# MrTornado24/FENeRF

Measured on NVIDIA H100. Metric: rendered faces/sec at 128px x 24 samples/ray, higher is better.
Workload: dtype f16 operands / f32 accumulate (wgmma) + f32 refinement

## Files before the change

fenerf_b200/_lib.py:

```python
import ctypes as C
import os

_HERE = os.path.dirname(os.path.abspath(__file__))
LIB_PATH = os.environ.get("FENERF_B200_LIB") or os.path.join(_HERE, "libfenerf_b200.so")

MAX_TRUNK, MAX_COLOR, MAX_LABEL, HIDDEN = 8, 8, 32, 256

ABI_VERSION = 3
FIELD_LABEL_FILM = 0x1
FIELD_FEATURE_HEAD = 0x8
PRECISION = {"exact": 0, "fast": 1, "guard": 2}
CLAMP = {"relu": 0, "softplus": 1}
FILL_MODE = {None: 0, "debug": 1, "weight": 2, "weight_debug": 3, "seg_padding_background": 4,
             "eval_seg_padding_background": 5, "eval_white_back": 6}
FILL_COLOR = {"black": 0.0, "white": 1.0, "grey": 0.5, "light_grey": 0.81}
E_CLAMP_MODE = -5
CAMERA_MODE = {"uniform": 1, "normal": 2, "gaussian": 2, "truncated_gaussian": 3, "spherical_uniform": 4}

EXPORTS = (
    "fenerf_packed_bytes", "fenerf_pack_field", "fenerf_siren_points", "fenerf_ray_setup", "fenerf_resample",
    "fenerf_composite", "fenerf_workspace_bytes", "fenerf_render_forward", "fenerf_last_error",
    "fenerf_abi_version", "fenerf_launch_count", "fenerf_camera_poses",
    "fenerf_field_fingerprint", "fenerf_composite_backward", "fenerf_film_forward_stash", "fenerf_gate_backward",
    "fenerf_head_grads", "fenerf_extras_gather", "fenerf_grid_scatter_add", "fenerf_grid_unpack_grad",
    "fenerf_workspace_layout", "fenerf_mask2color", "fenerf_frames_to_u8", "fenerf_mapping_film",
    "fenerf_guard_stats", "fenerf_debug_stage_times", "fenerf_gemm_nt_f16", "fenerf_gemm_nt_film", "fenerf_gemm_tn_f16",
)


class FieldDesc(C.Structure):
    _fields_ = [("trunk_layers", C.c_int32), ("color_layers", C.c_int32), ("label_dim", C.c_int32),
                ("grid_channels", C.c_int32), ("grid_res", C.c_int32), ("out_dim", C.c_int32),
                ("input_scale", C.c_float), ("reserved", C.c_int32)]


class FieldParams(C.Structure):
    _fields_ = [("trunk_w", C.c_void_p * MAX_TRUNK), ("trunk_b", C.c_void_p * MAX_TRUNK),
                ("sigma_w", C.c_void_p), ("sigma_b", C.c_void_p),
                ("color_w", C.c_void_p * MAX_COLOR), ("color_b", C.c_void_p * MAX_COLOR),
                ("rgb_w", C.c_void_p), ("rgb_b", C.c_void_p),
                ("label_w", C.c_void_p * 3), ("label_b", C.c_void_p * 3),
                ("grid", C.c_void_p)]


class RenderDesc(C.Structure):
    _fields_ = [("batch", C.c_int32), ("img_h", C.c_int32), ("img_w", C.c_int32), ("num_steps", C.c_int32),
                ("hierarchical", C.c_int32), ("clamp_mode", C.c_int32),
                ("last_back", C.c_int32), ("white_back", C.c_int32), ("black_back", C.c_int32),
                ("fill_mode", C.c_int32), ("fill_color", C.c_float), ("softmax_label", C.c_int32),
                ("lock_view_dependence", C.c_int32), ("precision", C.c_int32),
                ("noise_std", C.c_float), ("tan_half_fov", C.c_float), ("guard_tau", C.c_float)]


class GuardReport(C.Structure):
    _fields_ = [("refined", C.c_int32), ("max_abs_delta", C.c_float), ("sign_flips", C.c_int32), ("tau", C.c_float)]


class MappingParams(C.Structure):
    _fields_ = [("weight", C.c_void_p * 5), ("bias", C.c_void_p * 5), ("z_dim", C.c_int32), ("hidden_dim", C.c_int32)]
# ... 24 lines not shown
    lib.fenerf_ray_setup.argtypes = [P(RenderDesc)] + [vp] * 10
    lib.fenerf_resample.restype = C.c_int
    lib.fenerf_resample.argtypes = [P(RenderDesc), i32] + [vp] * 10
    lib.fenerf_composite.restype = C.c_int
    lib.fenerf_composite.argtypes = [P(RenderDesc), i32] + [vp] * 11
    lib.fenerf_workspace_bytes.restype = sz
    lib.fenerf_workspace_bytes.argtypes = [P(RenderDesc), P(FieldDesc)]
    lib.fenerf_workspace_layout.restype = C.c_int
    lib.fenerf_workspace_layout.argtypes = [P(RenderDesc), P(FieldDesc), P(WorkspaceOffsets)]
    lib.fenerf_render_forward.restype = C.c_int
    lib.fenerf_render_forward.argtypes = [P(RenderDesc), P(FieldDesc)] + [vp] * 15 + [vp, sz, vp]
    lib.fenerf_composite_backward.restype = C.c_int
    lib.fenerf_composite_backward.argtypes = [P(RenderDesc), i32] + [vp] * 9
    lib.fenerf_film_forward_stash.restype = C.c_int
    lib.fenerf_film_forward_stash.argtypes = [vp, vp, vp, i64, i64, i64, vp, i32, vp, vp, vp, i32, vp]
    lib.fenerf_gate_backward.restype = C.c_int
    lib.fenerf_gate_backward.argtypes = [vp, vp, i64, i64, vp, i32, vp]
    lib.fenerf_head_grads.restype = C.c_int
    lib.fenerf_head_grads.argtypes = [vp, vp, i64, i32, i32, vp, vp, vp, i32, vp]
    lib.fenerf_extras_gather.restype = C.c_int
    lib.fenerf_extras_gather.argtypes = [P(FieldDesc), vp, vp, vp, i64, i64, i32, i32, vp, vp]
    lib.fenerf_grid_scatter_add.restype = C.c_int
    lib.fenerf_grid_scatter_add.argtypes = [P(FieldDesc), vp, vp, i32, i64, vp, i32, vp]
    lib.fenerf_grid_unpack_grad.restype = C.c_int
    lib.fenerf_grid_unpack_grad.argtypes = [P(FieldDesc), vp, vp, vp, vp]
    lib.fenerf_gemm_nt_f16.restype = C.c_int
    lib.fenerf_gemm_nt_f16.argtypes = [vp, vp, i64, vp, vp, vp, vp]
    lib.fenerf_gemm_nt_film.restype = C.c_int
    lib.fenerf_gemm_nt_film.argtypes = [vp, vp, i64, vp, vp, i64, i64, vp, vp, vp, vp, vp]
    lib.fenerf_gemm_tn_f16.restype = C.c_int
    lib.fenerf_gemm_tn_f16.argtypes = [vp, vp, i32, i64, i32, vp, vp, vp]
    lib.fenerf_debug_stage_times.restype = C.c_int
    lib.fenerf_debug_stage_times.argtypes = [i32, vp]
    lib.fenerf_guard_stats.restype = C.c_int
    lib.fenerf_guard_stats.argtypes = [vp, P(GuardReport), vp]
    lib.fenerf_mapping_film.restype = C.c_int
    lib.fenerf_mapping_film.argtypes = [P(MappingParams), vp, i32, i32, i32, i32, vp, vp, C.c_float, vp, vp, vp]
    lib.fenerf_mask2color.restype = C.c_int
    lib.fenerf_mask2color.argtypes = [vp, i32, i32, i64, vp, vp]
    lib.fenerf_frames_to_u8.restype = C.c_int
    lib.fenerf_frames_to_u8.argtypes = [vp, i32, i32, i32, i32, i64, vp, vp]
    lib.fenerf_last_error.restype = C.c_char_p
    lib.fenerf_last_error.argtypes = []
    lib.fenerf_abi_version.restype = i32
    lib.fenerf_abi_version.argtypes = []
    lib.fenerf_launch_count.restype = i64
    lib.fenerf_launch_count.argtypes = []


def lib():
    global _lib
    if _lib is None:
        if not os.path.exists(LIB_PATH):
            raise RuntimeError(
                "libfenerf_b200.so is missing (%s): run `python -m fenerf_b200.build` or "
                "__graft_entry__.build(); the render path has no CPU / PyTorch fallback" % LIB_PATH)
        handle = C.CDLL(LIB_PATH)
        _declare(handle)
        if handle.fenerf_abi_version() != ABI_VERSION:
            raise RuntimeError("libfenerf_b200.so ABI version mismatch")
        _lib = handle
    return _lib


class FenerfError(RuntimeError):
    def __init__(self, code, message):
# ... 15 lines not shown
```

fenerf_b200/csrc/abi.cu:

```cuda
#include "common.cuh"
#include <stdlib.h>

namespace fn {
thread_local char g_err[512] = "";
std::atomic<long long> g_launches{0};
}

using namespace fn;

namespace {

struct Workspace {
    size_t stats, points_c, z_c, dirs, origins, raw_c, z_f, points_f, raw_f, guard, sigma_c, total;
};

Workspace plan_workspace(const fenerf_render_desc* rd, int C) {
    Workspace w;
    size_t n_rays = (size_t)rd->batch * rd->img_h * rd->img_w;
    size_t pc = n_rays * rd->num_steps;
    size_t off = 0;
    auto take = [&](size_t bytes) { size_t o = off; off = fn_align_up(off + bytes, 256); return o; };
    w.stats = take(64);
    w.points_c = take(pc * 3 * 4);
    w.z_c = take(pc * 4);
// ... 146 lines not shown
}

int fenerf_composite(const fenerf_render_desc* rd, int32_t out_dim, const float* raw_coarse, const float* z_coarse,
                     const float* raw_fine, const float* z_fine, const float* rng_noise, float* pixels, float* depth,
                     float* weights_sum, float* weights, int32_t* sort_idx, void* stream) {
    if (int e = check_render_desc(rd)) return e;
    FN_REQUIRE(raw_coarse && z_coarse && pixels, "NULL argument");
    FN_REQUIRE(rd->noise_std == 0.f || rng_noise, "noise_std != 0 needs rng_noise");
    return composite(rd, out_dim, raw_coarse, z_coarse, raw_fine, z_fine, rd->noise_std != 0.f ? rng_noise : nullptr,
                     pixels, depth, weights_sum, weights, sort_idx, (cudaStream_t)stream);
}

size_t fenerf_workspace_bytes(const fenerf_render_desc* rd, const fenerf_field_desc* field) {
    if (!rd || !field) return 0;
    return plan_workspace(rd, field->out_dim).total;
}

int fenerf_debug_stage_times(int32_t enable, float* ms_out) {
    if (enable && !g_stage_timing) {
        for (int i = 0; i <= kStages; ++i) FN_CUDA_OK(cudaEventCreate(&g_stage_ev[i]));
        g_stage_timing = true;
        return 0;
    }
    if (!enable && g_stage_timing) {
        g_stage_timing = false;
        for (int i = 0; i <= kStages; ++i) cudaEventDestroy(g_stage_ev[i]);
        return 0;
    }
    if (g_stage_timing && ms_out) {
        FN_CUDA_OK(cudaEventSynchronize(g_stage_ev[kStages]));
        for (int i = 0; i < kStages; ++i) FN_CUDA_OK(cudaEventElapsedTime(ms_out + i, g_stage_ev[i], g_stage_ev[i + 1]));
    }
    return 0;
}

int fenerf_guard_stats(const void* workspace, fenerf_guard_report* out, void* stream) {
    FN_REQUIRE(workspace && out, "NULL argument");
    int32_t raw[4];
    FN_CUDA_OK(cudaMemcpyAsync(raw, workspace, sizeof(raw), cudaMemcpyDeviceToHost, (cudaStream_t)stream));
    FN_CUDA_OK(cudaStreamSynchronize((cudaStream_t)stream));
    out->refined = raw[0];
    out->max_abs_delta = *reinterpret_cast<const float*>(&raw[1]);
    out->sign_flips = raw[2];
    out->tau = *reinterpret_cast<const float*>(&raw[3]);
    return 0;
}

int fenerf_workspace_layout(const fenerf_render_desc* rd, const fenerf_field_desc* field, fenerf_workspace_offsets* out) {
    if (int e = check_render_desc(rd)) return e;
    FN_REQUIRE(field && out, "NULL argument");
    Workspace w = plan_workspace(rd, field->out_dim);
    out->points_coarse = w.points_c; out->z_coarse = w.z_c; out->dirs = w.dirs; out->origins = w.origins;
    out->raw_coarse = w.raw_c; out->z_fine = w.z_f; out->points_fine = w.points_f; out->raw_fine = w.raw_f;
    out->total = w.total;
    return 0;
}

int fenerf_render_forward(const fenerf_render_desc* rd, const fenerf_field_desc* field, const void* packed,
                          const float* film, const float* x_lin, const float* y_lin, const float* z_lin,
                          const float* cam2world, const float* rng_perturb, const float* rng_noise_c,
                          const float* rng_u, const float* rng_noise_f, float* pixels, float* depth,
                          float* weights_sum, float* weights, int64_t* inds_dbg, void* workspace,
                          size_t workspace_bytes, void* stream) {
    if (int e = check_render_desc(rd)) return e;
    FnLayout L;
    FnLabelFilm lf;
// ... 173 lines not shown
```

fenerf_b200/csrc/common.cuh:

```cuda
#pragma once
#include <cuda_runtime.h>
#include <cuda_fp16.h>
#include <stdarg.h>
#include <stdint.h>
#include <stdio.h>
#include <atomic>

#include "../../include/fenerf_b200.h"
#include "layout.h"

namespace fn {

extern thread_local char g_err[512];
extern std::atomic<long long> g_launches;

inline int fail(int code, const char* fmt, ...) {
    va_list ap;
    va_start(ap, fmt);
    vsnprintf(g_err, sizeof(g_err), fmt, ap);
    va_end(ap);
    return code;
}

inline void count_launch(int n = 1) { g_launches.fetch_add(n, std::memory_order_relaxed); }
// ... 44 lines not shown
    const int dev = current_device();
    if (state[dev].load(std::memory_order_acquire) >= bytes) return cudaSuccess;
    cudaError_t e = cudaFuncSetAttribute(kernel, cudaFuncAttributeMaxDynamicSharedMemorySize, bytes);
    if (e == cudaSuccess) state[dev].store(bytes, std::memory_order_release);
    return e;
}

constexpr float kFarDelta = 1e10f;

__device__ __forceinline__ float softplus_torch(float x) { return x > 20.f ? x : log1pf(expf(x)); }

__device__ __forceinline__ float density_act(float sigma, int clamp_mode) {
    return clamp_mode == FENERF_CLAMP_RELU ? fmaxf(sigma, 0.f) : softplus_torch(sigma);
}

__device__ __forceinline__ float sample_alpha(float delta, float act, float* decay = nullptr) {
    const float e = expf(__fmul_rn(-delta, act));
    if (decay) *decay = e;
    return __fsub_rn(1.f, e);
}

__device__ __forceinline__ float transmittance_term(float alpha) { return __fadd_rn(__fsub_rn(1.f, alpha), 1e-10f); }

int pack_field(const fenerf_field_desc* f, const FnLayout& L, const FnLabelFilm& lf, const FnFeatureHead& fh,
               const fenerf_field_params* p, void* packed, cudaStream_t st);
int siren_points_exact(const FnLayout& L, const FnLabelFilm& lf, const FnFeatureHead& fh, const unsigned char* packed,
                       const float* points, const float* dirs, const float* film, int batch, long long ppb, int dir_group,
                       int lock_dirs, const int32_t* only_idx, int n_only, float* out, cudaStream_t st, int sigma_only = 0);
int field_fingerprint(const FnLayout& L, const FnLabelFilm& lf, const FnFeatureHead& fh, const fenerf_field_params* p,
                      unsigned long long* out, cudaStream_t st);
int siren_points_fast(const FnLayout& L, const FnLabelFilm& lf, const FnFeatureHead& fh, const unsigned char* packed,
                      const float* points, const float* dirs, const float* film, int batch, long long ppb, int dir_group,
                      int lock_dirs, float* out, int sigma_only, cudaStream_t st, float* sigma_out = nullptr);
int guard_refine(const FnLayout& L, const unsigned char* packed, const float* points, const float* dirs,
                 const float* film, int batch, long long rays_per_batch, int num_steps, int lock_dirs, float tau,
                 const float* noise_far, long long noise_stride, float noise_std,
                 float* raw, int32_t* scratch_idx, int32_t* stats, cudaStream_t st);
int camera_poses(int n, int mode, float h_std, float v_std, float h_mean, float v_mean, const float* draw_theta,
                 const float* draw_phi, float* c2w, float* pitch, float* yaw, cudaStream_t st);
int ray_setup(const fenerf_render_desc* rd, const float* x_lin, const float* y_lin, const float* z_lin,
              const float* cam2world, const float* rng_perturb, float* points, float* z_vals, float* dirs,
              float* origins, cudaStream_t st);
int resample(const fenerf_render_desc* rd, int C, const float* raw, const float* z, const float* dirs,
             const float* origins, const float* noise, const float* u, float* z_fine, float* pts_fine,
             long long* inds, cudaStream_t st, int sort_fine = 0, const float* sigma_compact = nullptr);
int composite_sorted(const fenerf_render_desc* rd, int C, const float* raw_c, const float* z_c, const float* raw_f,
                     const float* z_f, const float* noise, float* pixels, float* depth, float* wsum, float* weights,
                     cudaStream_t st);
int composite(const fenerf_render_desc* rd, int C, const float* raw_c, const float* z_c, const float* raw_f,
              const float* z_f, const float* noise, float* pixels, float* depth, float* wsum, float* weights,
              int32_t* sort_idx, cudaStream_t st);
int composite_backward(const fenerf_render_desc* rd, int C, const float* raw_c, const float* z_c, const float* raw_f,
                       const float* z_f, const float* noise, const float* d_pixels, float* d_raw_c, float* d_raw_f,
                       cudaStream_t st);

int gemm_nt(const void* A, const void* B, long long M, float* c32, void* c16, void* a_out, void* gate_out, const float* bias,
            const float* film, long long film_stride, long long ppb, cudaStream_t st, const void* gate_mul = nullptr,
            const void* A2 = nullptr, const void* B2 = nullptr);
int gemm_tn(const void* X, const void* Y, int batch, long long ppb, int slices, float* partial, cudaStream_t st,
            float* colsum = nullptr);
int mapping_film(const float* const* w, const float* const* b, const float* z, int B, int z_dim, int n_layers, int layer0,
                 int n_film_total, const float* avg_f, const float* avg_p, float psi, float* h_scratch, float* film,
                 cudaStream_t st);
int mask2color(const float* masks, int B, int K, long long HW, float* out, cudaStream_t st);
int frames_to_u8(const float* frames, int B, int C, int c0, int nc, long long HW, unsigned char* out, cudaStream_t st);
int film_forward_stash(const float* z, const float* bias, const float* film_layer, long long film_batch_stride, long long P,
// ... 13 lines not shown
```

fenerf_b200/csrc/siren_fast.cu:

```cuda
#include "siren_fast.cuh"

namespace fn {

int siren_fast_label_launch(const void* args, int blocks, cudaStream_t st);
int siren_fast_hd_launch(const void* args, int blocks, bool label_film, cudaStream_t st);

namespace {

bool build_loads(const FnLayout& L, const FnLabelFilm& lf, const FnFeatureHead& fh, FastArgs& A, bool sigma_only) {
    A.n_loads = 0;
    auto push = [&](size_t src, uint32_t bytes) {
        if (A.n_loads < MAX_LOADS) A.loads[A.n_loads] = Load{(uint32_t)src, bytes};
        ++A.n_loads;
    };
    push(L.first_img, 2 * CHUNK);
    for (int l = 0; l < L.n_hidden; ++l) {
        if (l == L.trunk_hidden) {
            push(L.head_img, 4 * HEAD_CHUNK);
            if (sigma_only) return A.n_loads <= MAX_LOADS;
        }
        if (lf.on && l == lf.layer) {
            push(L.hid_img[l], 2 * CHUNK);
            push(L.hid_img[l] + 2 * CHUNK, 2 * CHUNK);
            if (fh.on) push(fh.label_img, 4 * FEAT_CHUNK);
            else push(lf.img, 4 * HEAD_CHUNK);
            push(L.hid_img[l] + 4 * CHUNK, 2 * CHUNK);
            push(L.hid_img[l] + 6 * CHUNK, 2 * CHUNK);
            continue;
        }
        push(L.hid_img[l], 2 * CHUNK);
        push(L.hid_img[l] + 2 * CHUNK, 2 * CHUNK);
        if (l == L.trunk_hidden + lf.on) push(L.color0_ximg, 2 * CHUNK);
        push(L.hid_img[l] + 4 * CHUNK, 2 * CHUNK);
        push(L.hid_img[l] + 6 * CHUNK, 2 * CHUNK);
    }
    if (fh.on) push(fh.rgb_img, 4 * FEAT_CHUNK);
    else push(L.rgb_img, 4 * RGB_CHUNK);
    return A.n_loads <= MAX_LOADS;
}

}

int siren_points_fast(const FnLayout& L_in, const FnLabelFilm& lf_in, const FnFeatureHead& fh_in, const unsigned char* packed,
                      const float* points, const float* dirs, const float* film, int batch, long long ppb, int dir_group,
                      int lock_dirs, float* out, int sigma_only, cudaStream_t st, float* sigma_out) {
    static_assert(sizeof(FastArgs) <= 4000, "kernel parameter block too large");
    static_assert(SMEM_TOTAL <= 232448, "one CTA per SM: 227 KB of shared memory");
    static_assert(4 * FEAT_CHUNK == SLOT_BYTES, "a feature-head image is one ring slot");
    const FnFeatureHead no_fh = {0, 0, 0, 0, 0};
    const FnLabelFilm no_lf = {0, 0, 0};
    const bool trunk_only = fh_in.on && sigma_only;
    const FnFeatureHead& fh = trunk_only ? no_fh : fh_in;
    const FnLabelFilm& lf = trunk_only ? no_lf : lf_in;
    const FnLayout L = fh.on ? fn_head_view(L_in, fh) : fn_trunk_view(L_in, fh_in);
    FN_REQUIRE(L.trunk_hidden >= 1 && L.n_hidden - L.trunk_hidden - lf.on >= 1, "field needs >= 2 trunk and >= 1 colour layers");
    FN_REQUIRE(fh.on || L.label_dim < 32, "the fast path packs labels and sigma into one 32-column head (label_dim <= 31)");
    FN_REQUIRE(L.rgb_img < 0xFFFFFFFFull && lf.img < 0xFFFFFFFFull && fh.rgb_img < 0xFFFFFFFFull && fh.label_img < 0xFFFFFFFFull,
               "packed weight images beyond 4 GB");
    FN_REQUIRE(((uintptr_t)film & 15) == 0, "the FiLM table must be 16-byte aligned");
    FastArgs a;
    memset(&a, 0, sizeof(a));
    FN_REQUIRE(build_loads(L, lf, fh, a, sigma_only != 0), "field too deep for the weight stream");
    a.sigma_only = sigma_only ? 1 : 0;
    a.L = L; a.packed = packed; a.points = points; a.dirs = dirs; a.film = film; a.out = out; a.sigma_out = sigma_out;
    a.ppb = ppb; a.tiles_per_batch = (ppb + TILE - 1) / TILE; a.n_tiles = a.tiles_per_batch * batch;
    a.dir_group = dir_group < 1 ? 1 : dir_group; a.lock_dirs = lock_dirs;
    if (a.n_tiles <= 0) return 0;
    FN_REQUIRE(ppb % a.dir_group == 0, "points_per_batch %lld not a multiple of dir_group %d", ppb, a.dir_group);
    const long long n_pairs = (a.n_tiles + 1) / 2;
    static std::atomic<int> attr_set[kMaxDevices];
    const int blocks = (int)(n_pairs < (long long)num_sms() ? n_pairs : (long long)num_sms());
    if (fh.on) return siren_fast_hd_launch(&a, blocks, lf.on != 0, st);
    if (lf.on) return siren_fast_label_launch(&a, blocks, st);
    FN_CUDA_OK(ensure_dynamic_smem(siren_fast_kernel<false>, attr_set, (int)SMEM_TOTAL));
    siren_fast_kernel<false><<<blocks, NTHREADS, SMEM_TOTAL, st>>>(a);
    FN_LAUNCH_OK("siren_fast_kernel");
    return 0;
}

}
```

fenerf_b200/csrc/siren_fast.cuh:

```cuda
#pragma once
#include "common.cuh"
#include "siren_common.cuh"
#include "sm90.cuh"

namespace fn {

namespace {

using namespace sm90;

constexpr int TILE = 64;
constexpr int NTHREADS = 384;
constexpr int PROD_WARP = 8;
constexpr int RING = 6;
constexpr uint32_t SLOT_BYTES = 32768;
constexpr int XSTRIDE = 72;
constexpr uint32_t SMEM_X = RING * SLOT_BYTES;
constexpr int FRING = 2;
constexpr uint32_t FILM_BYTES = 3 * FN_H * 4;
constexpr uint32_t SMEM_FILM = SMEM_X + 2 * TILE * XSTRIDE * 2;
constexpr uint32_t SMEM_BAR = SMEM_FILM + 2 * FRING * FILM_BYTES;
constexpr uint32_t SMEM_TOTAL = SMEM_BAR + 16 * RING + 16 + 16 * 2 * FRING;
constexpr int MAX_LOADS = 72;
constexpr uint32_t CHUNK = 16384;
constexpr uint32_t HEAD_CHUNK = 32 * 128;
constexpr uint32_t RGB_CHUNK = 8 * 128;
constexpr uint32_t FEAT_CHUNK = FN_FEAT * 128;

struct Load {
    uint32_t src;
    uint32_t bytes;
};

struct FastArgs {
    Load loads[MAX_LOADS];
    int n_loads;
    FnLayout L;
    const unsigned char* packed;
    const float* points;
    const float* dirs;
    const float* film;
    float* out;
    float* sigma_out;
    long long ppb, tiles_per_batch, n_tiles;
    int dir_group, lock_dirs;
    int sigma_only;
};

__device__ __forceinline__ void wg_bar(int wg) { asm volatile("bar.sync %0, 128;" ::"r"(1 + wg) : "memory"); }

template <bool kLabelFilm, bool kFeatureHead = false>
__global__ void __launch_bounds__(NTHREADS, 1) siren_fast_kernel(const __grid_constant__ FastArgs a) {
    extern __shared__ __align__(1024) unsigned char smem[];
    const uint32_t sbase = smem_u32(smem);
    const int warp = threadIdx.x >> 5, lane = threadIdx.x & 31;
    const uint32_t bar_full = sbase + SMEM_BAR, bar_empty = bar_full + 8 * RING, bar_turn = bar_empty + 8 * RING;
    const uint32_t bar_ffull = bar_turn + 16, bar_fempty = bar_ffull + 8 * 2 * FRING;
    if (threadIdx.x == 0) {
        for (int i = 0; i < RING; ++i) {
            mbar_init(bar_full + 8 * i, 1);
            mbar_init(bar_empty + 8 * i, 8);
        }
        for (int g = 0; g < 2; ++g) mbar_init(bar_turn + 8 * g, 4);
        for (int e = 0; e < 2 * FRING; ++e) {
            mbar_init(bar_ffull + 8 * e, 1);
            mbar_init(bar_fempty + 8 * e, 4);
        }
        fence_barrier_init();
    }
    __syncthreads();
    const long long n_pairs = (a.n_tiles + 1) / 2;

    if (warp >= PROD_WARP) {
        asm volatile("setmaxnreg.dec.sync.aligned.u32 40;\n" ::: "memory");
        if (warp == PROD_WARP && lane == 0) {
            uint32_t it = 0;
            for (long long pair = blockIdx.x; pair < n_pairs; pair += gridDim.x)
                for (int i = 0; i < a.n_loads; ++i, ++it) {
                    const uint32_t slot = it % RING;
                    mbar_wait(bar_empty + 8 * slot, ((it / RING) & 1u) ^ 1u);
                    mbar_arrive_expect_tx(bar_full + 8 * slot, a.loads[i].bytes);
                    bulk_g2s(sbase + slot * SLOT_BYTES, a.packed + a.loads[i].src, a.loads[i].bytes, bar_full + 8 * slot);
                }
        } else if ((warp == PROD_WARP + 1 || warp == PROD_WARP + 2) && lane == 0) {
            const int g = warp - PROD_WARP - 1;
            const int n_film = 1 + (a.sigma_only ? a.L.trunk_hidden : a.L.n_hidden);
            uint32_t it = 0;
            for (long long pair = blockIdx.x; pair < n_pairs; pair += gridDim.x) {
                const long long tile = pair * 2 + g;
                const long long b = tile < a.n_tiles ? tile / a.tiles_per_batch : 0;
                const float* film_b = a.film + (size_t)b * a.L.n_film * 2 * FN_H;
                for (int i = 0; i < n_film; ++i, ++it) {
                    const uint32_t e = g * FRING + it % FRING;
                    const uint32_t dst = sbase + SMEM_FILM + e * FILM_BYTES;
                    mbar_wait(bar_fempty + 8 * e, ((it / FRING) & 1u) ^ 1u);
                    mbar_arrive_expect_tx(bar_ffull + 8 * e, FILM_BYTES);
                    bulk_g2s(dst, film_b + (size_t)i * 2 * FN_H, 2 * FN_H * 4, bar_ffull + 8 * e);
                    bulk_g2s(dst + 2 * FN_H * 4, a.packed + (i == 0 ? a.L.first_b : a.L.hid_b[i - 1]), FN_H * 4, bar_ffull + 8 * e);
                }
            }
        }
        return;
    }

    asm volatile("setmaxnreg.inc.sync.aligned.u32 232;\n" ::: "memory");
    const int wg = warp >> 2, q = lane & 3;
    const int tid = threadIdx.x & 127;
    const int r0 = (warp & 3) * 16 + (lane >> 2);
    const FnLayout& L = a.L;
    const int C = L.out_dim;
    const float* sigma_w = reinterpret_cast<const float*>(a.packed + L.sigma_w);
    const float* rgb_w = reinterpret_cast<const float*>(a.packed + L.rgb_w);
    const float* label_w = reinterpret_cast<const float*>(a.packed + L.label_w);
    __half* xs = reinterpret_cast<__half*>(smem + SMEM_X) + wg * TILE * XSTRIDE;
    uint32_t it = 0;
    auto acquire = [&](uint32_t& slot) -> uint32_t {
        slot = it % RING;
        mbar_wait(bar_full + 8 * slot, (it / RING) & 1u);
        ++it;
        return sbase + slot * SLOT_BYTES;
    };
    auto release = [&](uint32_t slot) {
        __syncwarp();
        if (lane == 0) mbar_arrive(bar_empty + 8 * slot);
    };
    uint32_t turns = 0;
    uint32_t fit = 0;
    auto film_acquire = [&]() -> const float* {
        const uint32_t e = wg * FRING + fit % FRING;
        mbar_wait(bar_ffull + 8 * e, (fit / FRING) & 1u);
        return reinterpret_cast<const float*>(smem + SMEM_FILM + e * FILM_BYTES);
    };
    auto film_release = [&]() {
        const uint32_t e = wg * FRING + fit % FRING;
        ++fit;
        __syncwarp();
        if (lane == 0) mbar_arrive(bar_fempty + 8 * e);
    };
    auto turn_begin = [&]() { mbar_wait(bar_turn + 8 * wg, (turns & 1u) ^ (wg == 0 ? 1u : 0u)); };
    auto turn_end = [&]() {
        ++turns;
        __syncwarp();
        if (lane == 0) mbar_arrive(bar_turn + 8 * (wg ^ 1));
    };
    auto xfrag = [&](int s, uint32_t (&f)[4]) {
        const __half* p = xs + r0 * XSTRIDE + 16 * s + 2 * q;
        f[0] = *reinterpret_cast<const uint32_t*>(p);
        f[1] = *reinterpret_cast<const uint32_t*>(p + 8 * XSTRIDE);
        f[2] = *reinterpret_cast<const uint32_t*>(p + 8);
        f[3] = *reinterpret_cast<const uint32_t*>(p + 8 * XSTRIDE + 8);
    };

    for (long long pair = blockIdx.x; pair < n_pairs; pair += gridDim.x) {
        const long long tile = pair * 2 + wg;
        const bool tile_ok = tile < a.n_tiles;
        const long long b = tile_ok ? tile / a.tiles_per_batch : 0;
        const long long p0 = tile_ok ? (tile % a.tiles_per_batch) * TILE : a.ppb;

        wg_bar(wg);
        if (tid < TILE) {
            float pos[3] = {0.f, 0.f, 0.f}, dir[3] = {0.f, 0.f, 0.f};
            const long long pp = p0 + tid;
            const bool valid = pp < a.ppb;
            if (valid) {
                const long long ff = b * a.ppb + pp;
#pragma unroll
                for (int i = 0; i < 3; ++i) pos[i] = __fmul_rn(a.points[ff * 3 + i], L.input_scale);
                if (a.lock_dirs) dir[2] = -1.f;
                else {
                    const long long di = b * (a.ppb / a.dir_group) + pp / a.dir_group;
#pragma unroll
                    for (int i = 0; i < 3; ++i) dir[i] = a.dirs[di * 3 + i];
                }
            }
            __align__(16) __half slots[64];
#pragma unroll
            for (int i = 0; i < 64; ++i) slots[i] = __float2half_rn(0.f);
#pragma unroll
            for (int i = 0; i < 3; ++i) {
                __half hi, lo;
                split_f16(pos[i], hi, lo);
                slots[FN_SLOT_POS + i] = hi; slots[FN_SLOT_POS + 3 + i] = lo; slots[FN_SLOT_POS + 6 + i] = hi;
                split_f16(dir[i], hi, lo);
                slots[FN_SLOT_DIR + i] = hi; slots[FN_SLOT_DIR + 3 + i] = lo; slots[FN_SLOT_DIR + 6 + i] = hi;
            }
            if (L.grid_channels > 0 && valid && !a.sigma_only) {
                float feat[32];
                grid_features32_h(reinterpret_cast<const __half*>(a.packed + L.grid16), L.grid_res, pos[0], pos[1], pos[2], feat);
#pragma unroll
                for (int i = 0; i < 32; ++i) slots[FN_SLOT_FEAT + i] = __float2half_rn(feat[i]);
            }
#pragma unroll
            for (int i = 0; i < 8; ++i)
                reinterpret_cast<uint4*>(xs + tid * XSTRIDE)[i] = reinterpret_cast<const uint4*>(slots)[i];
        }
        wg_bar(wg);

        uint32_t act[16][4];
        uint32_t nxt[8][4];
        float d[64];
        auto film_epi = [&](const float* fs, int h, uint32_t (&dst)[8][4]) {
            const float* fl = fs + h * 128;
            const float* bias = fs + 2 * FN_H + h * 128;
#pragma unroll
            for (int j = 0; j < 16; ++j) {
                const int c = 8 * j + 2 * q;
                const float2 fr = *reinterpret_cast<const float2*>(fl + c);
                const float2 ph = *reinterpret_cast<const float2*>(fl + FN_H + c);
                const float2 bi = *reinterpret_cast<const float2*>(bias + c);
                const float px = fmaf(fr.x, bi.x, ph.x), py = fmaf(fr.y, bi.y, ph.y);
                dst[j >> 1][(j & 1) * 2] = pack_half2(__sinf(fmaf(fr.x, d[4 * j], px)), __sinf(fmaf(fr.y, d[4 * j + 1], py)));
                dst[j >> 1][(j & 1) * 2 + 1] = pack_half2(__sinf(fmaf(fr.x, d[4 * j + 2], px)), __sinf(fmaf(fr.y, d[4 * j + 3], py)));
            }
        };
        auto act_hi = [&]() -> uint32_t (&)[8][4] { return *reinterpret_cast<uint32_t (*)[8][4]>(&act[8]); };

        {
            uint32_t xf[4], slot;
            const float* fs = nullptr;
            xfrag(0, xf);
            const uint32_t w = acquire(slot);
#pragma unroll
            for (int h = 0; h < 2; ++h) {
                turn_begin();
                wg_fence();
                mma_rs_n128(d, xf, desc_kmajor(w + h * CHUNK), 0u);
                wg_commit();
                turn_end();
                wg_wait<0>();
                fence_regs(d);
                fence_regs(xf);
                if (h == 0) fs = film_acquire();
                if (h == 0) film_epi(fs, 0, nxt);
                else film_epi(fs, 1, act_hi());
            }
            release(slot);
            film_release();
#pragma unroll
            for (int s = 0; s < 8; ++s)
#pragma unroll
                for (int i = 0; i < 4; ++i) act[s][i] = nxt[s][i];
        }

        bool stop = false;
        for (int l = 0; l < L.n_hidden && !stop; ++l) {
            if (l == L.trunk_hidden) {
                float dh[16];
                uint32_t slot;
                const uint32_t w = acquire(slot);
                turn_begin();
                wg_fence();
#pragma unroll
                for (int c = 0; c < 4; ++c)
#pragma unroll
                    for (int k = 0; k < 4; ++k) mma_rs_n32(dh, act[4 * c + k], desc_kmajor(w + c * HEAD_CHUNK + 32 * k), (c | k) ? 1u : 0u);
                wg_commit();
                turn_end();
                wg_wait<0>();
                fence_regs(dh);
                fence_regs(act);
                release(slot);
                const float inv_scale = L.label_dim > 0 ? __ldg(label_w + FENERF_MAX_LABEL * FN_H + FENERF_MAX_LABEL) : 1.f;
                const float* lb = label_w + FENERF_MAX_LABEL * FN_H;
#pragma unroll
                for (int rr = 0; rr < 2; ++rr) {
                    const long long pnt = p0 + r0 + 8 * rr;
                    if (pnt >= a.ppb) continue;
                    const long long flat = b * a.ppb + pnt;
#pragma unroll
                    for (int i = 0; i < 4; ++i)
#pragma unroll
                        for (int e = 0; e < 2; ++e) {
                            const int o = 8 * i + 2 * q + e;
                            const float v = dh[4 * i + 2 * rr + e];
                            if (!kFeatureHead && o < L.label_dim) {
                                if (!kLabelFilm && !a.sigma_only) a.out[flat * C + o] = fmaf(v, inv_scale, __ldg(lb + o));
                            } else if (o == (kFeatureHead ? 0 : L.label_dim)) {
                                const float sig = v + __ldg(sigma_w + FN_H);
                                a.out[flat * C + (C - 1)] = sig;
                                if (a.sigma_out) a.sigma_out[flat] = sig;
                            }
                        }
                }
                if (a.sigma_only) { stop = true; break; }
                if constexpr (kLabelFilm) {
                    constexpr int kLabN = kFeatureHead ? FN_FEAT : 32;
                    constexpr uint32_t kLabChunk = kFeatureHead ? FEAT_CHUNK : HEAD_CHUNK;
                    float dl[kLabN / 2];
                    uint32_t slot_h = 0, w_h = 0;
                    const float* fs = nullptr;
#pragma unroll
                    for (int h = 0; h < 2; ++h) {
                        uint32_t sl[2];
                        turn_begin();
                        wg_fence();
#pragma unroll
                        for (int sb = 0; sb < 2; ++sb) {
                            const uint32_t w = acquire(sl[sb]);
#pragma unroll
                            for (int c = 0; c < 2; ++c)
#pragma unroll
                                for (int k = 0; k < 4; ++k)
                                    mma_rs_n128(d, act[8 * sb + 4 * c + k], desc_kmajor(w + c * CHUNK + 32 * k), (sb | c | k) ? 1u : 0u);
                        }
                        wg_commit();
                        turn_end();
                        wg_wait<0>();
                        fence_regs(d);
                        fence_regs(act);
                        release(sl[0]);
                        release(sl[1]);
                        if (h == 0) fs = film_acquire();
                        film_epi(fs, h, nxt);
                        if (h == 0) w_h = acquire(slot_h);
                        turn_begin();
                        wg_fence();
#pragma unroll
                        for (int s = 0; s < 8; ++s) {
                            const int g = 8 * h + s;
                            const uint64_t desc = desc_kmajor(w_h + (g >> 2) * kLabChunk + 32 * (g & 3));
                            if constexpr (kFeatureHead) mma_rs_n64(dl, nxt[s], desc, (h | s) ? 1u : 0u);
                            else mma_rs_n32(dl, nxt[s], desc, (h | s) ? 1u : 0u);
                        }
                        wg_commit();
                        turn_end();
                        wg_wait<0>();
                        fence_regs(dl);
                        fence_regs(nxt);
                    }
                    release(slot_h);
                    film_release();
#pragma unroll
                    for (int rr = 0; rr < 2; ++rr) {
                        const long long pnt = p0 + r0 + 8 * rr;
                        if (pnt >= a.ppb) continue;
                        const long long flat = b * a.ppb + pnt;
                        const float* lbias = kFeatureHead ? label_w + FN_FEAT * FN_H : lb;
#pragma unroll
                        for (int i = 0; i < kLabN / 8; ++i)
#pragma unroll
                            for (int e = 0; e < 2; ++e) {
                                const int o = 8 * i + 2 * q + e;
                                if (o < L.label_dim) a.out[flat * C + o] = dl[4 * i + 2 * rr + e] + __ldg(lbias + o);
                            }
                    }
                    continue;
                }
            }
            const bool c0 = (l == L.trunk_hidden + (kLabelFilm ? 1 : 0));
            const int nx = L.grid_channels > 0 ? 3 : 1;
            uint32_t xf[3][4];
            if (c0)
#pragma unroll
                for (int s = 0; s < 3; ++s) xfrag(1 + s, xf[s]);
            uint32_t slot_x = 0, w_x = 0;
            const float* fs = nullptr;
#pragma unroll
            for (int h = 0; h < 2; ++h) {
                uint32_t sl[2];
                turn_begin();
                wg_fence();
#pragma unroll
                for (int sb = 0; sb < 2; ++sb) {
                    const uint32_t w = acquire(sl[sb]);
#pragma unroll
                    for (int c = 0; c < 2; ++c)
#pragma unroll
                        for (int k = 0; k < 4; ++k)
                            mma_rs_n128(d, act[8 * sb + 4 * c + k], desc_kmajor(w + c * CHUNK + 32 * k), (sb | c | k) ? 1u : 0u);
                }
                if (c0) {
                    if (h == 0) w_x = acquire(slot_x);
#pragma unroll
                    for (int s = 0; s < 3; ++s)
                        if (s < nx) mma_rs_n128(d, xf[s], desc_kmajor(w_x + h * CHUNK + 32 * (1 + s)), 1u);
                }
                wg_commit();
                turn_end();
                wg_wait<0>();
                fence_regs(d);
                fence_regs(act);
                fence_regs(xf);
                release(sl[0]);
                release(sl[1]);
                if (c0 && h == 1) release(slot_x);
                if (h == 0) fs = film_acquire();
                if (h == 0) film_epi(fs, 0, nxt);
                else film_epi(fs, 1, act_hi());
            }
            film_release();
#pragma unroll
            for (int s = 0; s < 8; ++s)
#pragma unroll
                for (int i = 0; i < 4; ++i) act[s][i] = nxt[s][i];
        }
        if (stop) continue;

        if constexpr (kFeatureHead) {
            float dr[32];
            uint32_t slot;
            const uint32_t w = acquire(slot);
            turn_begin();
            wg_fence();
#pragma unroll
            for (int c = 0; c < 4; ++c)
#pragma unroll
                for (int k = 0; k < 4; ++k) mma_rs_n64(dr, act[4 * c + k], desc_kmajor(w + c * FEAT_CHUNK + 32 * k), (c | k) ? 1u : 0u);
            wg_commit();
            turn_end();
            wg_wait<0>();
            fence_regs(dr);
            fence_regs(act);
            release(slot);
#pragma unroll
            for (int rr = 0; rr < 2; ++rr) {
                const long long pnt = p0 + r0 + 8 * rr;
                if (pnt >= a.ppb) continue;
                const long long flat = b * a.ppb + pnt;
#pragma unroll
                for (int i = 0; i < 8; ++i)
#pragma unroll
                    for (int e = 0; e < 2; ++e) {
                        const int o = 8 * i + 2 * q + e;
                        a.out[flat * C + L.label_dim + o] = dr[4 * i + 2 * rr + e] + __ldg(rgb_w + FN_FEAT * FN_H + o);
                    }
            }
            continue;
        }
        {
            float dr[4];
            uint32_t slot;
            const uint32_t w = acquire(slot);
            turn_begin();
            wg_fence();
#pragma unroll
            for (int c = 0; c < 4; ++c)
#pragma unroll
                for (int k = 0; k < 4; ++k) mma_rs_n8(dr, act[4 * c + k], desc_kmajor(w + c * RGB_CHUNK + 32 * k), (c | k) ? 1u : 0u);
            wg_commit();
            turn_end();
            wg_wait<0>();
            fence_regs(dr);
            fence_regs(act);
            release(slot);
#pragma unroll
            for (int rr = 0; rr < 2; ++rr) {
                const long long pnt = p0 + r0 + 8 * rr;
                if (pnt >= a.ppb) continue;
                const long long flat = b * a.ppb + pnt;
#pragma unroll
                for (int e = 0; e < 2; ++e) {
                    const int o = 2 * q + e;
                    if (o < 3) {
                        const float x = dr[2 * rr + e] + __ldg(rgb_w + 3 * FN_H + o);
                        a.out[flat * C + L.label_dim + o] = __fdividef(1.f, 1.f + __expf(-x));
                    }
                }
            }
        }
    }
}

}

}
```

include/fenerf_b200.h:

```cpp
#ifndef FENERF_B200_H
#define FENERF_B200_H

#include <stddef.h>
#include <stdint.h>

#ifdef __cplusplus
extern "C" {
#endif

#define FENERF_ABI_VERSION 3

#define FENERF_OK            0
#define FENERF_E_ARG        -1
#define FENERF_E_UNSUPPORTED -2
#define FENERF_E_CUDA       -3
#define FENERF_E_WORKSPACE  -4
#define FENERF_E_CLAMP_MODE -5

#define FENERF_MAX_TRUNK 8
#define FENERF_MAX_COLOR 8
#define FENERF_MAX_LABEL 32
#define FENERF_HIDDEN 256

#define FENERF_FIELD_LABEL_FILM 0x1
// ... 155 lines not shown
                       float* colsum, void* stream);

int fenerf_composite_backward(const fenerf_render_desc* rd, int32_t out_dim, const float* raw_coarse,
                              const float* z_coarse, const float* raw_fine, const float* z_fine,
                              const float* rng_noise, const float* d_pixels,
                              float* d_raw_coarse, float* d_raw_fine, void* stream);

int fenerf_film_forward_stash(const float* z, const float* bias, const float* film_layer, int64_t film_batch_stride,
                              int64_t n_points, int64_t points_per_batch, const float* narrow_in, int32_t narrow_width,
                              const float* narrow_w, void* a_out, void* gate_out, int32_t dtype, void* stream);

int fenerf_gate_backward(void* dA, const void* gate, int64_t n_points, int64_t points_per_batch, float* colsum,
                         int32_t dtype, void* stream);

int fenerf_head_grads(const float* d_raw, const float* raw, int64_t n_points, int32_t out_dim, int32_t label_dim,
                      const float* scale, void* d_heads, void* d_rgb, int32_t dtype, void* stream);

int fenerf_extras_gather(const fenerf_field_desc* field, const void* packed, const float* points, const float* dirs,
                         int64_t n_points, int64_t points_per_batch, int32_t dir_group, int32_t lock_dirs, float* out,
                         void* stream);

int fenerf_grid_scatter_add(const fenerf_field_desc* field, const float* points, const void* d_feat, int32_t ld,
                            int64_t n_points, float* grad_channels_last, int32_t dtype, void* stream);
int fenerf_grid_unpack_grad(const fenerf_field_desc* field, const float* grad_channels_last, float* out,
                            const float* inv_scale, void* stream);

const char* fenerf_last_error(void);

int32_t fenerf_abi_version(void);
int64_t fenerf_launch_count(void);

int fenerf_debug_stage_times(int32_t enable, float* ms_out );

#ifdef __cplusplus
}
#endif
#endif
```

Measured before the change: 578.8.

## Precompute FiLM phase-plus-bias in loader warps and add debug tracing variants

The FiLM loader warps now compute freq*bias+phase and store interleaved float4 (freq, phase') per channel pair, so the compute epilogue does one vectorised smem load per pair instead of three float2 loads plus an FMA. The loader goes from lane-0 bulk copies to all 32 lanes doing __ldg and stores, with the film-full barrier now counting 32 arrivals. The smem FiLM slot shrinks from three rows to two. Also adds optional debug-only variants: per-warp clock64 timeline tracing and a polynomial software sine that offloads part of the MUFU sine work to FMA; both are off by default.

```diff
diff --git a/fenerf_b200/_lib.py b/fenerf_b200/_lib.py
--- a/fenerf_b200/_lib.py
+++ b/fenerf_b200/_lib.py
@@ -24,7 +24,8 @@
     "fenerf_field_fingerprint", "fenerf_composite_backward", "fenerf_film_forward_stash", "fenerf_gate_backward",
     "fenerf_head_grads", "fenerf_extras_gather", "fenerf_grid_scatter_add", "fenerf_grid_unpack_grad",
     "fenerf_workspace_layout", "fenerf_mask2color", "fenerf_frames_to_u8", "fenerf_mapping_film",
-    "fenerf_guard_stats", "fenerf_debug_stage_times", "fenerf_gemm_nt_f16", "fenerf_gemm_nt_film", "fenerf_gemm_tn_f16",
+    "fenerf_guard_stats", "fenerf_debug_stage_times", "fenerf_debug_fast_variant", "fenerf_debug_soft_sine",
+    "fenerf_gemm_nt_f16", "fenerf_gemm_nt_film", "fenerf_gemm_tn_f16",
 )
 
 
@@ -115,6 +116,10 @@
     lib.fenerf_gemm_tn_f16.argtypes = [vp, vp, i32, i64, i32, vp, vp, vp]
     lib.fenerf_debug_stage_times.restype = C.c_int
     lib.fenerf_debug_stage_times.argtypes = [i32, vp]
+    lib.fenerf_debug_fast_variant.restype = C.c_int
+    lib.fenerf_debug_fast_variant.argtypes = [i32, vp, i32]
+    lib.fenerf_debug_soft_sine.restype = C.c_int
+    lib.fenerf_debug_soft_sine.argtypes = [vp, vp, i64, vp]
     lib.fenerf_guard_stats.restype = C.c_int
     lib.fenerf_guard_stats.argtypes = [vp, P(GuardReport), vp]
     lib.fenerf_mapping_film.restype = C.c_int
diff --git a/fenerf_b200/csrc/abi.cu b/fenerf_b200/csrc/abi.cu
--- a/fenerf_b200/csrc/abi.cu
+++ b/fenerf_b200/csrc/abi.cu
@@ -202,6 +202,15 @@
         for (int i = 0; i < kStages; ++i) FN_CUDA_OK(cudaEventElapsedTime(ms_out + i, g_stage_ev[i], g_stage_ev[i + 1]));
     }
     return 0;
+}
+
+int fenerf_debug_fast_variant(int32_t variant, void* trace, int32_t trace_ctas) {
+    return siren_fast_debug_variant(variant, static_cast<unsigned long long*>(trace), trace_ctas);
+}
+
+int fenerf_debug_soft_sine(const float* a, float* out, int64_t n, void* stream) {
+    FN_REQUIRE(a && out && n >= 0, "bad argument");
+    return soft_sine_eval(a, out, n, (cudaStream_t)stream);
 }
 
 int fenerf_guard_stats(const void* workspace, fenerf_guard_report* out, void* stream) {
diff --git a/fenerf_b200/csrc/common.cuh b/fenerf_b200/csrc/common.cuh
--- a/fenerf_b200/csrc/common.cuh
+++ b/fenerf_b200/csrc/common.cuh
@@ -100,6 +100,8 @@
 int siren_points_fast(const FnLayout& L, const FnLabelFilm& lf, const FnFeatureHead& fh, const unsigned char* packed,
                       const float* points, const float* dirs, const float* film, int batch, long long ppb, int dir_group,
                       int lock_dirs, float* out, int sigma_only, cudaStream_t st, float* sigma_out = nullptr);
+int siren_fast_debug_variant(int variant, unsigned long long* trace, int trace_ctas);
+int soft_sine_eval(const float* a, float* out, long long n, cudaStream_t st);
 int guard_refine(const FnLayout& L, const unsigned char* packed, const float* points, const float* dirs,
                  const float* film, int batch, long long rays_per_batch, int num_steps, int lock_dirs, float tau,
                  const float* noise_far, long long noise_stride, float noise_std,
diff --git a/fenerf_b200/csrc/siren_fast.cu b/fenerf_b200/csrc/siren_fast.cu
--- a/fenerf_b200/csrc/siren_fast.cu
+++ b/fenerf_b200/csrc/siren_fast.cu
@@ -4,8 +4,13 @@
 
 int siren_fast_label_launch(const void* args, int blocks, cudaStream_t st);
 int siren_fast_hd_launch(const void* args, int blocks, bool label_film, cudaStream_t st);
+int siren_fast_debug_launch(const void* args, int blocks, bool label_film, bool feature_head, int variant, cudaStream_t st);
 
 namespace {
+
+std::atomic<int> g_variant{0};
+unsigned long long* g_trace = nullptr;
+int g_trace_ctas = 0;
 
 bool build_loads(const FnLayout& L, const FnLabelFilm& lf, const FnFeatureHead& fh, FastArgs& A, bool sigma_only) {
     A.n_loads = 0;
@@ -41,6 +46,15 @@
 
 }
 
+int siren_fast_debug_variant(int variant, unsigned long long* trace, int trace_ctas) {
+    FN_REQUIRE(variant >= 0 && variant <= 3, "unknown point-network variant %d", variant);
+    FN_REQUIRE(variant < 2 || (trace && trace_ctas >= 1), "a timeline variant needs its trace buffer");
+    g_trace = trace;
+    g_trace_ctas = trace_ctas;
+    g_variant.store(variant);
+    return 0;
+}
+
 int siren_points_fast(const FnLayout& L_in, const FnLabelFilm& lf_in, const FnFeatureHead& fh_in, const unsigned char* packed,
                       const float* points, const float* dirs, const float* film, int batch, long long ppb, int dir_group,
                       int lock_dirs, float* out, int sigma_only, cudaStream_t st, float* sigma_out) {
@@ -70,6 +84,11 @@
     const long long n_pairs = (a.n_tiles + 1) / 2;
     static std::atomic<int> attr_set[kMaxDevices];
     const int blocks = (int)(n_pairs < (long long)num_sms() ? n_pairs : (long long)num_sms());
+    if (const int variant = g_variant.load()) {
+        a.trace = g_trace;
+        a.trace_ctas = g_trace_ctas;
+        return siren_fast_debug_launch(&a, blocks, lf.on != 0, fh.on != 0, variant, st);
+    }
     if (fh.on) return siren_fast_hd_launch(&a, blocks, lf.on != 0, st);
     if (lf.on) return siren_fast_label_launch(&a, blocks, st);
     FN_CUDA_OK(ensure_dynamic_smem(siren_fast_kernel<false>, attr_set, (int)SMEM_TOTAL));
diff --git a/fenerf_b200/csrc/siren_fast.cuh b/fenerf_b200/csrc/siren_fast.cuh
--- a/fenerf_b200/csrc/siren_fast.cuh
+++ b/fenerf_b200/csrc/siren_fast.cuh
@@ -17,7 +17,7 @@
 constexpr int XSTRIDE = 72;
 constexpr uint32_t SMEM_X = RING * SLOT_BYTES;
 constexpr int FRING = 2;
-constexpr uint32_t FILM_BYTES = 3 * FN_H * 4;
+constexpr uint32_t FILM_BYTES = 2 * FN_H * 4;
 constexpr uint32_t SMEM_FILM = SMEM_X + 2 * TILE * XSTRIDE * 2;
 constexpr uint32_t SMEM_BAR = SMEM_FILM + 2 * FRING * FILM_BYTES;
 constexpr uint32_t SMEM_TOTAL = SMEM_BAR + 16 * RING + 16 + 16 * 2 * FRING;
@@ -26,6 +26,33 @@
 constexpr uint32_t HEAD_CHUNK = 32 * 128;
 constexpr uint32_t RGB_CHUNK = 8 * 128;
 constexpr uint32_t FEAT_CHUNK = FN_FEAT * 128;
+#ifndef FENERF_SOFT_SIN_EVERY
+#define FENERF_SOFT_SIN_EVERY 0
+#endif
+constexpr int kSoftSinEvery = FENERF_SOFT_SIN_EVERY;
+constexpr int kSoftSinSplit = 4;
+constexpr int TRACE_CAP = 1024;
+constexpr int TRACE_WARPS = 11;
+enum TraceEvent {
+    TR_PAIR = 1, TR_TURN_WAIT, TR_TURN_DONE, TR_ACQ_WAIT, TR_ACQ_DONE, TR_COMMIT, TR_MMA_DONE, TR_EPI_DONE,
+    TR_FILM_WAIT, TR_FILM_DONE, TR_EMPTY_WAIT, TR_EMPTY_DONE,
+};
+enum TraceGroup { TG_FIRST = 0, TG_HIDDEN, TG_COLOR0, TG_TRUNK_HEAD, TG_LABEL_LAYER, TG_LABEL_HEAD, TG_OUT_HEAD };
+
+__device__ __forceinline__ float soft_sinf(float a) {
+    const float k = fmaf(a, 0.159154943f, 12582912.f);
+    const float n = k - 12582912.f;
+    float r = fmaf(-n, 6.28318548f, a);
+    r = fmaf(-n, -1.74845553e-7f, r);
+    const float r2 = r * r;
+    float p = -2.041572245e-08f;
+    p = fmaf(p, r2, 2.701100129e-06f);
+    p = fmaf(p, r2, -1.980991656e-04f);
+    p = fmaf(p, r2, 8.332454599e-03f);
+    p = fmaf(p, r2, -1.666656137e-01f);
+    p = fmaf(p, r2, 9.999996424e-01f);
+    return r * p;
+}
 
 struct Load {
     uint32_t src;
@@ -45,17 +72,29 @@
     long long ppb, tiles_per_batch, n_tiles;
     int dir_group, lock_dirs;
     int sigma_only;
+    unsigned long long* trace;
+    int trace_ctas;
 };
 
 __device__ __forceinline__ void wg_bar(int wg) { asm volatile("bar.sync %0, 128;" ::"r"(1 + wg) : "memory"); }
 
-template <bool kLabelFilm, bool kFeatureHead = false>
+template <bool kLabelFilm, bool kFeatureHead = false, int kSoftSin = kSoftSinEvery, bool kTrace = false>
 __global__ void __launch_bounds__(NTHREADS, 1) siren_fast_kernel(const __grid_constant__ FastArgs a) {
     extern __shared__ __align__(1024) unsigned char smem[];
     const uint32_t sbase = smem_u32(smem);
     const int warp = threadIdx.x >> 5, lane = threadIdx.x & 31;
     const uint32_t bar_full = sbase + SMEM_BAR, bar_empty = bar_full + 8 * RING, bar_turn = bar_empty + 8 * RING;
     const uint32_t bar_ffull = bar_turn + 16, bar_fempty = bar_ffull + 8 * 2 * FRING;
+    unsigned long long* tbuf = nullptr;
+    uint32_t tn = 0;
+    if constexpr (kTrace)
+        if (lane == 0 && (int)blockIdx.x < a.trace_ctas) tbuf = a.trace + ((size_t)blockIdx.x * TRACE_WARPS + warp) * TRACE_CAP;
+    auto trace = [&](int kind, int group = 0) {
+        if constexpr (kTrace)
+            if (tbuf && tn < TRACE_CAP)
+                tbuf[tn++] = ((unsigned long long)kind << 56) | ((unsigned long long)group << 48) |
+                             ((unsigned long long)clock64() & ((1ull << 48) - 1));
+    };
     if (threadIdx.x == 0) {
         for (int i = 0; i < RING; ++i) {
             mbar_init(bar_full + 8 * i, 1);
@@ -63,7 +102,7 @@
         }
         for (int g = 0; g < 2; ++g) mbar_init(bar_turn + 8 * g, 4);
         for (int e = 0; e < 2 * FRING; ++e) {
-            mbar_init(bar_ffull + 8 * e, 1);
+            mbar_init(bar_ffull + 8 * e, 32);
             mbar_init(bar_fempty + 8 * e, 4);
         }
         fence_barrier_init();
@@ -78,11 +117,13 @@
             for (long long pair = blockIdx.x; pair < n_pairs; pair += gridDim.x)
                 for (int i = 0; i < a.n_loads; ++i, ++it) {
                     const uint32_t slot = it % RING;
+                    trace(TR_EMPTY_WAIT);
                     mbar_wait(bar_empty + 8 * slot, ((it / RING) & 1u) ^ 1u);
+                    trace(TR_EMPTY_DONE);
                     mbar_arrive_expect_tx(bar_full + 8 * slot, a.loads[i].bytes);
                     bulk_g2s(sbase + slot * SLOT_BYTES, a.packed + a.loads[i].src, a.loads[i].bytes, bar_full + 8 * slot);
                 }
-        } else if ((warp == PROD_WARP + 1 || warp == PROD_WARP + 2) && lane == 0) {
+        } else if (warp == PROD_WARP + 1 || warp == PROD_WARP + 2) {
             const int g = warp - PROD_WARP - 1;
             const int n_film = 1 + (a.sigma_only ? a.L.trunk_hidden : a.L.n_hidden);
             uint32_t it = 0;
@@ -92,11 +133,19 @@
                 const float* film_b = a.film + (size_t)b * a.L.n_film * 2 * FN_H;
                 for (int i = 0; i < n_film; ++i, ++it) {
                     const uint32_t e = g * FRING + it % FRING;
-                    const uint32_t dst = sbase + SMEM_FILM + e * FILM_BYTES;
+                    const float2* row = reinterpret_cast<const float2*>(film_b + (size_t)i * 2 * FN_H);
+                    const float2* bias = reinterpret_cast<const float2*>(a.packed + (i == 0 ? a.L.first_b : a.L.hid_b[i - 1]));
+                    float4* dst = reinterpret_cast<float4*>(smem + SMEM_FILM + e * FILM_BYTES);
+                    trace(TR_EMPTY_WAIT);
                     mbar_wait(bar_fempty + 8 * e, ((it / FRING) & 1u) ^ 1u);
-                    mbar_arrive_expect_tx(bar_ffull + 8 * e, FILM_BYTES);
-                    bulk_g2s(dst, film_b + (size_t)i * 2 * FN_H, 2 * FN_H * 4, bar_ffull + 8 * e);
-                    bulk_g2s(dst + 2 * FN_H * 4, a.packed + (i == 0 ? a.L.first_b : a.L.hid_b[i - 1]), FN_H * 4, bar_ffull + 8 * e);
+                    trace(TR_EMPTY_DONE);
+#pragma unroll 1
+                    for (int k = 0; k < FN_H / 64; ++k) {
+                        const int cp = lane + 32 * k;
+                        const float2 f = __ldg(row + cp), p = __ldg(row + FN_H / 2 + cp), bb = __ldg(bias + cp);
+                        dst[cp] = make_float4(f.x, f.y, fmaf(f.x, bb.x, p.x), fmaf(f.y, bb.y, p.y));
+                    }
+                    mbar_arrive(bar_ffull + 8 * e);
                 }
             }
         }
@@ -116,7 +165,9 @@
     uint32_t it = 0;
     auto acquire = [&](uint32_t& slot) -> uint32_t {
         slot = it % RING;
+        trace(TR_ACQ_WAIT);
         mbar_wait(bar_full + 8 * slot, (it / RING) & 1u);
+        trace(TR_ACQ_DONE);
         ++it;
         return sbase + slot * SLOT_BYTES;
     };
@@ -126,10 +177,12 @@
     };
     uint32_t turns = 0;
     uint32_t fit = 0;
-    auto film_acquire = [&]() -> const float* {
+    auto film_acquire = [&]() -> const float4* {
         const uint32_t e = wg * FRING + fit % FRING;
+        trace(TR_FILM_WAIT);
         mbar_wait(bar_ffull + 8 * e, (fit / FRING) & 1u);
-        return reinterpret_cast<const float*>(smem + SMEM_FILM + e * FILM_BYTES);
+        trace(TR_FILM_DONE);
+        return reinterpret_cast<const float4*>(smem + SMEM_FILM + e * FILM_BYTES);
     };
     auto film_release = [&]() {
         const uint32_t e = wg * FRING + fit % FRING;
@@ -137,8 +190,13 @@
         __syncwarp();
         if (lane == 0) mbar_arrive(bar_fempty + 8 * e);
     };
-    auto turn_begin = [&]() { mbar_wait(bar_turn + 8 * wg, (turns & 1u) ^ (wg == 0 ? 1u : 0u)); };
-    auto turn_end = [&]() {
+    auto turn_begin = [&]() {
+        trace(TR_TURN_WAIT);
+        mbar_wait(bar_turn + 8 * wg, (turns & 1u) ^ (wg == 0 ? 1u : 0u));
+        trace(TR_TURN_DONE);
+    };
+    auto turn_end = [&](int group) {
+        trace(TR_COMMIT, group);
         ++turns;
         __syncwarp();
         if (lane == 0) mbar_arrive(bar_turn + 8 * (wg ^ 1));
@@ -156,6 +214,7 @@
         const bool tile_ok = tile < a.n_tiles;
         const long long b = tile_ok ? tile / a.tiles_per_batch : 0;
         const long long p0 = tile_ok ? (tile % a.tiles_per_batch) * TILE : a.ppb;
+        trace(TR_PAIR);
 
         wg_bar(wg);
         if (tid < TILE) {
@@ -199,25 +258,22 @@
         uint32_t act[16][4];
         uint32_t nxt[8][4];
         float d[64];
-        auto film_epi = [&](const float* fs, int h, uint32_t (&dst)[8][4]) {
-            const float* fl = fs + h * 128;
-            const float* bias = fs + 2 * FN_H + h * 128;
+        auto film_epi = [&](const float4* fs, int h, uint32_t (&dst)[8][4]) {
 #pragma unroll
             for (int j = 0; j < 16; ++j) {
-                const int c = 8 * j + 2 * q;
-                const float2 fr = *reinterpret_cast<const float2*>(fl + c);
-                const float2 ph = *reinterpret_cast<const float2*>(fl + FN_H + c);
-                const float2 bi = *reinterpret_cast<const float2*>(bias + c);
-                const float px = fmaf(fr.x, bi.x, ph.x), py = fmaf(fr.y, bi.y, ph.y);
-                dst[j >> 1][(j & 1) * 2] = pack_half2(__sinf(fmaf(fr.x, d[4 * j], px)), __sinf(fmaf(fr.y, d[4 * j + 1], py)));
-                dst[j >> 1][(j & 1) * 2 + 1] = pack_half2(__sinf(fmaf(fr.x, d[4 * j + 2], px)), __sinf(fmaf(fr.y, d[4 * j + 3], py)));
-            }
+                const float4 e = fs[64 * h + 4 * j + q];
+                const bool soft = kSoftSin > 0 && j % (kSoftSin > 0 ? kSoftSin : 1) == kSoftSin - 1;
+                auto sn = [soft](float x) { return soft ? soft_sinf(x) : __sinf(x); };
+                dst[j >> 1][(j & 1) * 2] = pack_half2(sn(fmaf(e.x, d[4 * j], e.z)), sn(fmaf(e.y, d[4 * j + 1], e.w)));
+                dst[j >> 1][(j & 1) * 2 + 1] = pack_half2(sn(fmaf(e.x, d[4 * j + 2], e.z)), sn(fmaf(e.y, d[4 * j + 3], e.w)));
+            }
+            trace(TR_EPI_DONE);
         };
         auto act_hi = [&]() -> uint32_t (&)[8][4] { return *reinterpret_cast<uint32_t (*)[8][4]>(&act[8]); };
 
         {
             uint32_t xf[4], slot;
-            const float* fs = nullptr;
+            const float4* fs = nullptr;
             xfrag(0, xf);
             const uint32_t w = acquire(slot);
 #pragma unroll
@@ -226,8 +282,9 @@
                 wg_fence();
                 mma_rs_n128(d, xf, desc_kmajor(w + h * CHUNK), 0u);
                 wg_commit();
-                turn_end();
+                turn_end(TG_FIRST);
                 wg_wait<0>();
+                trace(TR_MMA_DONE);
                 fence_regs(d);
                 fence_regs(xf);
                 if (h == 0) fs = film_acquire();
@@ -255,8 +312,9 @@
 #pragma unroll
                     for (int k = 0; k < 4; ++k) mma_rs_n32(dh, act[4 * c + k], desc_kmajor(w + c * HEAD_CHUNK + 32 * k), (c | k) ? 1u : 0u);
                 wg_commit();
-                turn_end();
+                turn_end(TG_TRUNK_HEAD);
                 wg_wait<0>();
+                trace(TR_MMA_DONE);
                 fence_regs(dh);
                 fence_regs(act);
                 release(slot);
@@ -288,7 +346,7 @@
                     constexpr uint32_t kLabChunk = kFeatureHead ? FEAT_CHUNK : HEAD_CHUNK;
                     float dl[kLabN / 2];
                     uint32_t slot_h = 0, w_h = 0;
-                    const float* fs = nullptr;
+                    const float4* fs = nullptr;
 #pragma unroll
                     for (int h = 0; h < 2; ++h) {
                         uint32_t sl[2];
@@ -304,8 +362,9 @@
                                     mma_rs_n128(d, act[8 * sb + 4 * c + k], desc_kmajor(w + c * CHUNK + 32 * k), (sb | c | k) ? 1u : 0u);
                         }
                         wg_commit();
-                        turn_end();
+                        turn_end(TG_LABEL_LAYER);
                         wg_wait<0>();
+                        trace(TR_MMA_DONE);
                         fence_regs(d);
                         fence_regs(act);
                         release(sl[0]);
@@ -323,8 +382,9 @@
                             else mma_rs_n32(dl, nxt[s], desc, (h | s) ? 1u : 0u);
                         }
                         wg_commit();
-                        turn_end();
+                        turn_end(TG_LABEL_HEAD);
                         wg_wait<0>();
+                        trace(TR_MMA_DONE);
                         fence_regs(dl);
                         fence_regs(nxt);
                     }
@@ -354,7 +414,7 @@
 #pragma unroll
                 for (int s = 0; s < 3; ++s) xfrag(1 + s, xf[s]);
             uint32_t slot_x = 0, w_x = 0;
-            const float* fs = nullptr;
+            const float4* fs = nullptr;
 #pragma unroll
             for (int h = 0; h < 2; ++h) {
                 uint32_t sl[2];
@@ -376,8 +436,9 @@
                         if (s < nx) mma_rs_n128(d, xf[s], desc_kmajor(w_x + h * CHUNK + 32 * (1 + s)), 1u);
                 }
                 wg_commit();
-                turn_end();
+                turn_end(c0 ? TG_COLOR0 : TG_HIDDEN);
                 wg_wait<0>();
+                trace(TR_MMA_DONE);
                 fence_regs(d);
                 fence_regs(act);
                 fence_regs(xf);
@@ -407,8 +468,9 @@
 #pragma unroll
                 for (int k = 0; k < 4; ++k) mma_rs_n64(dr, act[4 * c + k], desc_kmajor(w + c * FEAT_CHUNK + 32 * k), (c | k) ? 1u : 0u);
             wg_commit();
-            turn_end();
+            turn_end(TG_OUT_HEAD);
             wg_wait<0>();
+            trace(TR_MMA_DONE);
             fence_regs(dr);
             fence_regs(act);
             release(slot);
@@ -438,8 +500,9 @@
 #pragma unroll
                 for (int k = 0; k < 4; ++k) mma_rs_n8(dr, act[4 * c + k], desc_kmajor(w + c * RGB_CHUNK + 32 * k), (c | k) ? 1u : 0u);
             wg_commit();
-            turn_end();
+            turn_end(TG_OUT_HEAD);
             wg_wait<0>();
+            trace(TR_MMA_DONE);
             fence_regs(dr);
             fence_regs(act);
             release(slot);
diff --git a/fenerf_b200/csrc/siren_fast_debug.cu b/fenerf_b200/csrc/siren_fast_debug.cu
--- /dev/null
+++ b/fenerf_b200/csrc/siren_fast_debug.cu
@@ -0,0 +1,41 @@
+#include "siren_fast.cuh"
+
+namespace fn {
+
+namespace {
+
+template <bool kLabelFilm, bool kFeatureHead, int kSoftSin, bool kTrace>
+int launch(const FastArgs& a, int blocks, cudaStream_t st) {
+    static std::atomic<int> attr_set[kMaxDevices];
+    FN_CUDA_OK(ensure_dynamic_smem(siren_fast_kernel<kLabelFilm, kFeatureHead, kSoftSin, kTrace>, attr_set, (int)SMEM_TOTAL));
+    siren_fast_kernel<kLabelFilm, kFeatureHead, kSoftSin, kTrace><<<blocks, NTHREADS, SMEM_TOTAL, st>>>(a);
+    FN_LAUNCH_OK("siren_fast_kernel<debug>");
+    return 0;
+}
+
+__global__ void soft_sine_kernel(const float* a, float* out, long long n) {
+    const long long i = (long long)blockIdx.x * blockDim.x + threadIdx.x;
+    if (i < n) out[i] = soft_sinf(a[i]);
+}
+
+}
+
+int siren_fast_debug_launch(const void* args, int blocks, bool label_film, bool feature_head, int variant, cudaStream_t st) {
+    const FastArgs& a = *static_cast<const FastArgs*>(args);
+    if (variant == 1) {
+        if (feature_head) return label_film ? launch<true, true, kSoftSinSplit, false>(a, blocks, st) : launch<false, true, kSoftSinSplit, false>(a, blocks, st);
+        return label_film ? launch<true, false, kSoftSinSplit, false>(a, blocks, st) : launch<false, false, kSoftSinSplit, false>(a, blocks, st);
+    }
+    FN_REQUIRE(!label_film && !feature_head, "the point-network timeline covers plain fields only");
+    if (variant == 2) return launch<false, false, kSoftSinEvery, true>(a, blocks, st);
+    return launch<false, false, kSoftSinSplit, true>(a, blocks, st);
+}
+
+int soft_sine_eval(const float* a, float* out, long long n, cudaStream_t st) {
+    if (n <= 0) return 0;
+    soft_sine_kernel<<<(unsigned)((n + 255) / 256), 256, 0, st>>>(a, out, n);
+    FN_LAUNCH_OK("soft_sine_kernel");
+    return 0;
+}
+
+}
diff --git a/include/fenerf_b200.h b/include/fenerf_b200.h
--- a/include/fenerf_b200.h
+++ b/include/fenerf_b200.h
@@ -211,6 +211,9 @@
 
 int fenerf_debug_stage_times(int32_t enable, float* ms_out );
 
+int fenerf_debug_fast_variant(int32_t variant, void* trace, int32_t trace_ctas);
+int fenerf_debug_soft_sine(const float* a, float* out, int64_t n, void* stream);
+
 #ifdef __cplusplus
 }
 #endif
```

Result: faster. 600.7 (median of 6 runs) (+3.8%).
